# Illumina/strelka

Measured on AMD Instinct MI355X. Metric: candidate-alignment scoring cells/s (read bases x candidate alignments; Strelka2 has no pair-HMM, SURVEY.md section 0) + germline loci/s + 40x WGS-like germline wall-clock (e2e) + 110x/40x somatic wall-clock (e2e_somatic), higher is better.
Workload: dtype f64; 1 GPU; germline chr20-style synthetic (BASELINE.json configs[1]).  Headline: scoreCandidateAlignment as one function -- per GPU per step 65536 reads of 150 bp x 87.9 candidate alignments each (5-7 candidate indels around them), from the candidate alignments the device search left (PCal) to one double each: one kernel (F5: the walk of each alignment's path + the terms of its bases, penalties and clips).  ; read_len=150

## Files before the change

### include/strelka_amd.h

```cpp
#ifndef STRELKA_AMD_H
#define STRELKA_AMD_H

#include <stddef.h>
#include <stdint.h>

#ifdef __cplusplus
extern "C" {
#endif

#define SK_VERSION 100


int sk_device_count(void);
void* sk_host_alloc(size_t bytes);
void sk_host_free(void* p);
int sk_init(int device);
int sk_init_strict(int device);
void sk_shutdown(void);
const char* sk_last_error(void);
int sk_version(void);
int sk_is_initialized(void);
int sk_sync_mode(void);
int sk_libm_restated(void);

int sk_broker_client(void);
int sk_broker_enable(int on);
int sk_broker_serve(int device, const char* socket_name, int idle_seconds);
int sk_broker_selftest(int n, uint32_t mul);

int sk_check_device_errors(void);

int sk_debug_set_g3_variant(int variant);
int sk_debug_g3_global_pass_count(void);
int sk_debug_force_device_libm(int on);
void sk_debug_region_alleles(int no_edge_deletion, int ids_twice);

int sk_get_qscore_tables(double* q2p, double* q2lncompe, double* q2lne);


enum { SK_BAM_REF = 0, SK_BAM_A = 1, SK_BAM_C = 2, SK_BAM_G = 4, SK_BAM_T = 8, SK_BAM_ANY = 15 };

enum {
    SK_OP_BASES = 0,
    SK_OP_SOFT_CLIP = 1,
    SK_OP_NOBASE = 2
};
enum { SK_OPFLAG_NONCANDIDATE_PENALTY = 1 };

typedef struct sk_score_op {
    uint16_t length;
// ... 836 lines not shown
```

### strelka_amd/capi.py

```python
import ctypes as C
import os

import numpy as np

_HERE = os.path.dirname(os.path.abspath(__file__))
LIB_PATH = os.path.join(_HERE, "lib", "libstrelka_amd.so")

c_void_p = C.c_void_p


class ScoreOp(C.Structure):
    _fields_ = [("length", C.c_uint16), ("kind", C.c_uint8), ("flags", C.c_uint8), ("src", C.c_int32)]


SCORE_OP_DTYPE = np.dtype([("length", "<u2"), ("kind", "u1"), ("flags", "u1"), ("src", "<i4")])
OP_BASES, OP_SOFT_CLIP, OP_NOBASE = 0, 1, 2
OPFLAG_PENALTY = 1


class AlignBatch(C.Structure):
    _fields_ = [("n_reads", C.c_int32), ("n_cals", C.c_int32), ("n_ops", C.c_int64),
                ("read_off", c_void_p), ("read_code", c_void_p), ("read_qual", c_void_p),
                ("hap_off", c_void_p), ("hap_code", c_void_p), ("cal_off", c_void_p), ("op_off", c_void_p),
                ("ops", c_void_p), ("max_read_len", C.c_int32), ("max_hap_len", C.c_int32),
# ... 198 lines not shown
    "sk_score_alignments", "sk_score_alignments_dev", "sk_align_evmask_words", "sk_align_prepare", "sk_align_colmat_words", "sk_align_prepare_cols",
    "sk_bgzf_scan", "sk_bgzf_inflate", "sk_bgzf_inflate_prefixed", "sk_bgzf_inflate_dev", "sk_bgzf_deflate_bound", "sk_bgzf_deflate", "sk_bgzf_deflate_dev", "sk_bam_header_end", "sk_bam_scan_records", "sk_bam_decode", "sk_bam_decode_kept", "sk_bam_decode_dev", "sk_normalize_alignments", "sk_normalize_alignments_dev",
    "sk_intake_options_default", "sk_read_intake_obs_bound", "sk_read_intake", "sk_read_intake_dev", "sk_read_intake_scratch_bytes",
    "sk_ar_state_initial", "sk_ref_anchors", "sk_ref_anchors_dev", "sk_active_regions_bound", "sk_active_regions", "sk_active_regions_dev",
    "sk_region_haplotypes_seq_bound", "sk_region_haplotypes_support_bound", "sk_region_haplotypes_scratch_bytes", "sk_region_haplotypes", "sk_region_haplotypes_dev",
    "sk_region_alleles_allele_bound", "sk_region_alleles_insert_bound", "sk_region_alleles_scratch_bytes", "sk_region_alleles", "sk_region_alleles_dev", "sk_debug_region_alleles",
    "sk_align_builder_create", "sk_align_builder_destroy", "sk_align_builder_clear", "sk_align_builder_append", "sk_align_builder_add_read",
    "sk_align_builder_finish", "sk_align_builder_error", "sk_align_builder_set_host_threads",
    "sk_align_scores_default", "sk_global_align",
    "sk_pileup_options_default", "sk_pileup_reads", "sk_pileup_reads_dev", "sk_pileup_scratch_bytes",
    "sk_pileup_stream_create", "sk_pileup_stream_destroy", "sk_pileup_stream_begin_region", "sk_pileup_stream_push", "sk_pileup_stream_push_begin", "sk_pileup_stream_push_finish", "sk_pileup_stream_enable_evs_words", "sk_gvcf_site_summaries", "sk_gvcf_site_summaries_dev", "sk_gvcf_plain_runs_dev", "sk_gvcf_plain_runs", "sk_pileup_stream_set_gvcf_block_options",
    "sk_somatic_pileup_stream_create", "sk_somatic_pileup_stream_destroy", "sk_somatic_pileup_stream_begin_region", "sk_somatic_pileup_stream_push", "sk_somatic_pileup_stream_push_begin", "sk_somatic_pileup_stream_push_finish",
    "sk_realign_options_default", "sk_realign_job_create", "sk_realign_job_destroy", "sk_realign_job_error",
    "sk_realign_job_set_reference", "sk_realign_job_set_indels", "sk_realign_job_add_read", "sk_realign_job_add_reads", "sk_realign_job_get_batch",
    "sk_realign_job_finish", "sk_realign_job_run", "sk_realign_job_n_reads", "sk_realign_job_read_result",
    "sk_realign_job_clear_reads", "sk_realign_job_rescore", "sk_realign_job_indels_consulted", "sk_realign_job_enumeration_counts", "sk_realign_device_job_counts", "sk_realign_reference_reads_outside", "sk_realign_job_stage3_counts", "sk_make_start_pos_alignment", "sk_get_end_pin_start_pos",
    "sk_germline_options_default", "sk_dependent_eprob", "sk_dependent_eprob_dev", "sk_site_digt_call",
    "sk_site_digt_call_dev", "sk_site_digt_call_fused", "sk_site_digt_call_fused_dev",
    "sk_somatic_snv_options_default", "sk_somatic_snv_call_batch", "sk_somatic_snv_call_batch_dev",
    "sk_somatic_snv_call_tiers", "sk_somatic_snv_call_tiers_dev", "sk_somatic_snv_tiers_scratch_bytes",
    "sk_indel_options_default", "sk_somatic_indel_options_default", "sk_indel_grid_lhood", "sk_indel_grid_lhood_dev",
    "sk_somatic_indel_call_batch", "sk_somatic_indel_call_tiers", "sk_allele_group_genotype_lhoods", "sk_allele_group_genotype_lhoods_dev",
    "sk_allele_group_genotype_lhoods_wide", "sk_allele_group_genotype_lhoods_wide_dev",
    "sk_allele_group_genotype_lhoods_xwide", "sk_allele_group_genotype_lhoods_xwide_dev",
    "sk_discover_indels_and_mismatches", "sk_global_align_scratch_bytes", "sk_global_align_dev", "sk_bai_query", "sk_bam_region_filter", "sk_gvcf_block_sites", "sk_gvcf_block_sites_dev",
]

_lib = None


def lib():
# ... 19 lines not shown
        L.sk_align_scores_default.argtypes = [C.POINTER(AlignScores)]
        L.sk_global_align.argtypes = [C.POINTER(GlobalAlignBatch), C.POINTER(AlignScores), c_void_p, c_void_p, c_void_p, c_void_p]
        L.sk_pileup_options_default.argtypes = [C.POINTER(PileupOptions)]
        L.sk_pileup_reads.argtypes = [C.POINTER(ReadBatchStruct), C.POINTER(PileupOptions), C.c_int, C.POINTER(PileupColumns)]
        L.sk_pileup_scratch_bytes.restype = C.c_int64
        L.sk_pileup_scratch_bytes.argtypes = [C.c_int32, C.c_int64, C.c_int32]
        L.sk_pileup_reads_dev.argtypes = [C.POINTER(ReadBatchStruct), C.c_int64, C.POINTER(PileupOptions), C.c_int,
                                          C.POINTER(PileupColumns), c_void_p, c_void_p]
        L.sk_realign_options_default.argtypes = [C.POINTER(RealignOptions)]
        L.sk_realign_job_create.restype = c_void_p
        L.sk_realign_job_create.argtypes = [C.POINTER(RealignOptions)]
        L.sk_realign_job_destroy.argtypes = [c_void_p]
        L.sk_realign_job_enumeration_counts.argtypes = [c_void_p, c_void_p, c_void_p, c_void_p]
        L.sk_realign_device_job_counts.argtypes = [c_void_p, c_void_p, c_void_p]
        L.sk_realign_device_job_counts.restype = None
        L.sk_realign_reference_reads_outside.argtypes = []
        L.sk_realign_reference_reads_outside.restype = C.c_int64
        L.sk_realign_job_stage3_counts.argtypes = [c_void_p, c_void_p, c_void_p]
        L.sk_realign_job_indels_consulted.argtypes = [c_void_p, c_void_p, C.c_int32]
        L.sk_realign_job_error.restype = C.c_char_p
        L.sk_realign_job_error.argtypes = [c_void_p]
        L.sk_realign_job_set_reference.argtypes = [c_void_p, C.c_char_p, C.c_int32, C.c_int32]
        L.sk_realign_job_set_indels.argtypes = [c_void_p, C.POINTER(IndelInfo), C.c_int32]
        L.sk_realign_job_add_read.argtypes = [c_void_p, C.POINTER(ReadInput)]
        L.sk_realign_job_add_reads.argtypes = [c_void_p, C.POINTER(ReadInput), C.c_int32]
        L.sk_realign_job_get_batch.argtypes = [c_void_p, C.POINTER(AlignBatch)]
        L.sk_realign_job_finish.argtypes = [c_void_p, c_void_p]
        L.sk_realign_job_run.argtypes = [c_void_p]
        L.sk_realign_job_n_reads.argtypes = [c_void_p]
        L.sk_realign_job_read_result.argtypes = [c_void_p, C.c_int32, C.POINTER(ReadResult)]
# ... 682 lines not shown
        if lib().sk_realign_job_indels_consulted(self._j, _p(out), self._n_indels):
            raise self._err()
        return out[:self._n_indels]

    def enumeration_counts(self):
        a, b, c = C.c_int64(), C.c_int64(), C.c_int64()
        lib().sk_realign_job_enumeration_counts(self._j, C.byref(a), C.byref(b), C.byref(c))
        return a.value, b.value, c.value

    @staticmethod
    def device_job_counts():
        a, b, c = C.c_int64(), C.c_int64(), C.c_int64()
        lib().sk_realign_device_job_counts(C.byref(a), C.byref(b), C.byref(c))
        return a.value, b.value, c.value

    def stage3_counts(self):
        a, b = C.c_int64(), C.c_int64()
        lib().sk_realign_job_stage3_counts(self._j, C.byref(a), C.byref(b))
        return a.value, b.value

    def clear_reads(self):
        lib().sk_realign_job_clear_reads(self._j)

    def result(self, i):
        r = ReadResult()
        if lib().sk_realign_job_read_result(self._j, i, C.byref(r)):
            raise StrelkaAmdError("bad read index")
        scores = []
        for q in range(r.n_scores):
            s = r.scores[q]
# ... 696 lines not shown
```

### strelka_amd/csrc/read_enumerate.hip

```cpp

#include "sk_common.h"

#include "align_entry.h"
#include "read_enumerate.h"

#include <algorithm>
#include <chrono>
#include <climits>
#include <cstdio>
#include <cstdlib>
#include <cstring>
#include <vector>

using namespace skcore;

int sk_score_alignments_launch_hostleg(const sk_align_batch* b, double* dev_out_lnp, void* hip_stream);

namespace
{

static_assert(sizeof(PFrame) % 4 == 0 && sizeof(PCal) % 4 == 0, "frames move through LDS as 32-bit words");


struct EnumArgs
// ... 238 lines not shown


enum { DYN_N_GROUPED = 0, DYN_N_CALS, DYN_N_LIGHT, DYN_N_HEAVY, DYN_FLAGS, DYN_MAX_CALS, DYN_REF_OUTSIDE, DYN_COUNT = 8 };
enum { DYNF_DEEPER = 1,
       DYNF_POOL_FULL = 2 };
enum { SEARCH_LEVELS = Caps::K + 2,
       CNT_LEVELS = 0,
       CNT_LEAVES = Caps::K + 3,
       CNT_NODES = (Caps::K + 5) & ~1,
       CNT_UNHANDLED = Caps::K + 7,
       CNT_DYN = Caps::K + 8,
       CNT_QUEUE = CNT_DYN + DYN_COUNT,
       N_COUNTERS = CNT_QUEUE + 2 };
static_assert(CNT_LEVELS + SEARCH_LEVELS + 1 == CNT_LEAVES && CNT_NODES > CNT_LEAVES && CNT_NODES + 2 <= CNT_UNHANDLED, "the counters' slots overlap");

__device__ inline int block_exclusive_scan(const int v, int* wave_sums , int* total)
{
    const int lane = threadIdx.x & 63, wave = threadIdx.x >> 6, n_waves = blockDim.x >> 6;
    int x = v;
    for (int d = 1; d < 64; d <<= 1) {
        const int y = __shfl_up(x, d);
        if (lane >= d) x += y;
    }
    __syncthreads();
    if (lane == 63) wave_sums[wave] = x;
    __syncthreads();
    if (threadIdx.x == 0) {
        int run = 0;
        for (int w = 0; w < n_waves; ++w) {
            const int t = wave_sums[w];
            wave_sums[w] = run;
            run += t;
        }
        wave_sums[n_waves] = run;
    }
    __syncthreads();
    *total = wave_sums[n_waves];
    return wave_sums[wave] + x - v;
}

struct ScanArgs
{
    int32_t n_reads;
    const int32_t* status;
    const int32_t* count;
// ... 448 lines not shown
constexpr int F5_TAB = 32;

static_assert(F5_TAB <= 32, "the table copy is a lane an entry, the consulted mask a bit an entry");

struct FusedScoreArgs
{
    FlatArgs f;
    const uint8_t* read_qual;
    const SkTables* tab;
    double* scores;
    unsigned* err;
    int32_t* n_unhandled;
    int32_t write_cals;
    unsigned long long* dbg;
    unsigned* queue;
};

constexpr int F5_SEGS = 16, F5_INDELS = 8;
constexpr int F5_STAMPS = 9;
constexpr int F5_SLOT = (F5_SEGS + 1) | 1;
__device__ __forceinline__ int f5_ent_word(const int k) { return k; }
constexpr int F5_ROW = 3;

struct F5Tab
{
    int32_t pos;
    uint32_t del, ins_len;
    uint32_t type_cand;
    int32_t ins_at;
};

template <int MAXR>
struct F5Lds
{
// ... 604 lines not shown
        const unsigned long long td = now();
        stamp[4] += td - tc;
        if (has && !bad) {
            const double lnp = f5_sum(S, myslot, n_ent, ln_noncand, ln_quarter);
            fa.scores[c0 + my_j] = lnp;
        }
        if (cons_mine && cons_seen == 0) a.job.consulted[tab_lo + lane] = 1;
        raw0.q0 = raw0.q1 = raw0.q2 = raw0.q3 = raw0.q4 = make_uint4(0, 0, 0, 0);
        raw0.i0 = raw0.i1 = raw0.i2 = raw0.i3 = 0;
        stamp[5] += now() - td;
    }
    if (TIMING && fa.dbg && lane == 0) {
        stamp[6] = now();
        stamp[3] = TIMING ? (unsigned long long)wall_clock64() - wall0 : 0ull;
        stamp[8] = draw_cycles;
        for (int i = 0; i < F5_STAMPS; ++i) fa.dbg[size_t(r) * F5_STAMPS + i] = stamp[i];
    }
}

template <int MAXR, bool TIMING, int WAVES>
__global__ __launch_bounds__(64 * WAVES) __attribute__((amdgpu_waves_per_eu(4, 4))) void flatten_score_kernel(const FusedScoreArgs fa, const int n_reads)
{
    __shared__ __attribute__((aligned(16))) F5Lds<MAXR> S[WAVES];
    __shared__ double q_terms[F5_Q_TERMS];
    for (int i = threadIdx.x; i < F5_Q_TERMS; i += 64 * WAVES) q_terms[i] = (i <= SK_NQ) ? fa.tab->q2lncompe[i] : fa.tab->q2mis[i - (SK_NQ + 1)];
    __syncthreads();
    const int wave = threadIdx.x >> 6, lane = threadIdx.x & 63;
    const unsigned n_waves = gridDim.x * unsigned(WAVES);
    unsigned r = blockIdx.x * unsigned(WAVES) + unsigned(wave);
    unsigned long long draw_cycles = 0;
    while (r < unsigned(n_reads)) {
        f5_read<MAXR, TIMING>(fa, int(r), S[wave], q_terms, draw_cycles);
        f5_wave_sync();
        const unsigned long long t0 = TIMING ? (unsigned long long)clock64() : 0ull;
        unsigned d = 0;
        if (lane == 0) d = atomicAdd(&fa.queue[0], 1u);
        int drawn = __builtin_amdgcn_readfirstlane(int(d));
        if (TIMING) __asm__ volatile("" : "+s"(drawn));
        r = n_waves + unsigned(drawn);
        draw_cycles = TIMING ? (unsigned long long)clock64() - t0 : 0ull;
    }
    if (lane == 0) {
        __threadfence();
        if (atomicAdd(&fa.queue[1], 1u) == gridDim.x * unsigned(WAVES) - 1u) {
            fa.queue[0] = 0u;
            fa.queue[1] = 0u;
        }
    }
}

template <int MAXR, bool TIMING>
static void launch_flatten_score_t(const int n_reads, hipStream_t st, const FusedScoreArgs& fs)
{
    static const int waves = [] { const char* e = std::getenv("SK_F5_WAVES"); return e ? std::atoi(e) : 0; }();
    constexpr int DEFAULT_WAVES = (sizeof(F5Lds<MAXR>) * 16 <= 160 * 1024) ? 8 : 4;
    const int w = waves > 0 ? waves : DEFAULT_WAVES;
    static const int grid_env = [] { const char* e = std::getenv("SK_F5_GRID"); return e ? std::atoi(e) : 0; }();
    constexpr int WAVES_PER_CU = int((160 * 1024) / sizeof(F5Lds<MAXR>)) >= 16 ? 16 : int((160 * 1024) / sizeof(F5Lds<MAXR>));
    auto grid = [&](const int wpb) {
        const int resident = grid_env > 0 ? grid_env : 256 * std::max(1, WAVES_PER_CU / wpb);
        return dim3(unsigned(std::max(1, std::min(resident, (n_reads + wpb - 1) / wpb))));
    };
    if (w == 16 && MAXR <= 152) SK_LAUNCH((flatten_score_kernel<152, TIMING, 16>), grid(16), dim3(1024), 0, st, fs, n_reads);
    else if (w >= 8) SK_LAUNCH((flatten_score_kernel<MAXR, TIMING, 8>), grid(8), dim3(512), 0, st, fs, n_reads);
    else if (w == 4) SK_LAUNCH((flatten_score_kernel<MAXR, TIMING, 4>), grid(4), dim3(256), 0, st, fs, n_reads);
    else if (w == 2) SK_LAUNCH((flatten_score_kernel<MAXR, TIMING, 2>), grid(2), dim3(128), 0, st, fs, n_reads);
    else SK_LAUNCH((flatten_score_kernel<MAXR, TIMING, 1>), grid(1), dim3(64), 0, st, fs, n_reads);
}

static void launch_flatten_score(const int n_reads, hipStream_t st, const FusedScoreArgs& fs)
{
    const bool short_reads = fs.f.max_read_len <= 152, timing = fs.dbg != nullptr;
    if (short_reads && !timing) launch_flatten_score_t<152, false>(n_reads, st, fs);
    else if (short_reads) launch_flatten_score_t<152, true>(n_reads, st, fs);
    else if (!timing) launch_flatten_score_t<F5_MAX_READ, false>(n_reads, st, fs);
    else launch_flatten_score_t<F5_MAX_READ, true>(n_reads, st, fs);
}

__global__ __launch_bounds__(64) void gather_cals_kernel(const PCal* __restrict__ pool, const int32_t* __restrict__ list, const int32_t n_cals,
                                                         PCal* __restrict__ cals)
{
    constexpr int REC_DW = int(sizeof(PCal) / 4);
// ... 465 lines not shown

struct EnumBuffers
{
    DevBuf in_arena, zero_arena, minmax_arena, mask_arena;
    HostBuf h_in_arena, h_zero_arena;
    View tab, ins, toggle, ref, ref_code, ins_code, reads, read_off, read_code, read_qual, r2i, i2r, orig, map_level;
    View counters, status, warn, n_raw, hap_len, fill, n_uniq, consulted;
    View win_begin, ins_lo, win_end, ins_hi, evmask, addmask;
    View h_counters, h_status, h_warn, h_n_raw, h_hap_len, h_n_uniq, h_consulted;
    View cal_off_z, h_cal_off_z;
    DevBuf level_a, level_b, pool, leaf_read, leaf_hash;
    DevBuf raw_off, grouped, ghash, gkey, dup, sorted;
    DevBuf n_ops, win_len, n_ins, ins_idx, ins_off, n_seg8;
    DevBuf cal_off, hap_off, cals, hap_code, op_off, ops, entries, scores, colmat, colmat_off;
    DevBuf s3_order, s3_smooth, s3_flag, s3_rm_type, s3_rm_pos, s3_key, s3_sorted_score, s3_sorted_hash, s3_next_same, s3_range_end, s3_removed, s3_out, s3_list;
    HostBuf h_s3_out, h_s3_list;
    HostBuf h_raw_off, h_n_ops, h_cal_off, h_hap_off, h_op_off, h_cals, h_scores, h_colmat_off;
};
EnumBuffers& bufs()
{
    static EnumBuffers b;
    return b;
}

int reserve_dev(std::initializer_list<std::pair<DevBuf&, size_t>> wants)
{
    for (const auto& w : wants)
        if (w.first.reserve(std::max<size_t>(w.second, 256))) return 1;
    return 0;
}
// ... 60 lines not shown
    SK_HIP(skrt::setDevice(ctx.device));
    if (!g_cals_gathered) {
        if (bufs().cals.reserve(sizeof(PCal) * size_t(g_n_cals))) return 1;
        SK_LAUNCH(gather_cals_kernel, dim3((g_n_cals + 63) / 64), dim3(64), 0, ctx.stream, g_cals_pool, g_cals_list, g_n_cals, bufs().cals.as<PCal>());
        SK_HIP(skrt::getLastError());
        g_cals_gathered = true;
    }
    SK_HIP(skrt::memcpyAsync(dst, bufs().cals.as<PCal>() + first, sizeof(PCal) * size_t(count), hipMemcpyDeviceToHost, ctx.stream));
    SK_HIP(skrt::streamSynchronize(ctx.stream));
    return 0;
}

namespace
{
int64_t g_jobs_one_wait = 0, g_jobs_one_wait_redone = 0, g_jobs_staged = 0;
struct JobSeconds
{
    double setup = 0, submit = 0, wait = 0, after = 0;
    ~JobSeconds()
    {
        if (std::getenv("SK_ENUM_JOB_SECONDS"))
            std::fprintf(stderr, "strelka_amd enum job seconds: jobs=%lld setup=%.4f submit=%.4f wait=%.4f after=%.4f\n", (long long)g_jobs_one_wait, setup, submit,
                         wait, after);
    }
} g_job_seconds;
}
extern "C" void sk_enum_device_job_counts(int64_t* one_wait, int64_t* one_wait_redone, int64_t* staged)
{
    if (one_wait) *one_wait = g_jobs_one_wait;
    if (one_wait_redone) *one_wait_redone = g_jobs_one_wait_redone;
    if (staged) *staged = g_jobs_staged;
}

namespace
{
struct JobPlan
{
    const SkEnumInput* in = nullptr;
    EnumBuffers& B = bufs();
    hipStream_t st = nullptr;
    bool one_wait = false, with_stage3 = false;
    int n = 0;
    int64_t n_bases = 0, frame_cap = 0, pool_cap = 0;
    int W = 0;
    int max_order = 0;
    size_t in_bytes = 0, zero_bytes = 0, minmax_bytes = 0, mask_bytes = 0;
    size_t minmax_split = 0;
// ... 48 lines not shown
    if (one_wait && !(test_caps && test_caps[0])) p.pool_cap = std::min<int64_t>(p.pool_cap, std::max<int64_t>(int64_t(n) * 256, 1 << 17));
    const bool s3 = p.with_stage3 = in->want_scores && in->want_stage3;
    const int W = p.W = sk_ent_evmask_words(std::max(in->max_read_len, 0));
    for (int r = 0; r < n; ++r) p.max_order = std::max(p.max_order, int(in->reads[r].n_order));
    if (const char* e = std::getenv("SK_STAGE3_TEST_LDS_CALS")) {
        int a = 0, b = 0;
        if (std::sscanf(e, "%d,%d", &a, &b) == 2 && a > 0 && b >= a && b <= S3_LDS_CALS) {
            p.light_cals = a;
            p.lds_cals = b;
        }
    }
    if (reserve_dev({ { B.level_a, sizeof(PFrame) * size_t(p.frame_cap) }, { B.level_b, sizeof(PFrame) * size_t(p.frame_cap) },
                      { B.pool, sizeof(PCal) * size_t(p.pool_cap) }, { B.leaf_read, 4 * size_t(p.pool_cap) }, { B.leaf_hash, 4 * size_t(p.pool_cap) },
                      { B.raw_off, 4 * size_t(n + 1) }, { B.win_len, 4 * size_t(n) }, { B.n_ins, 4 * size_t(n) },
                      { B.ins_idx, 2 * size_t(n) * INS_CAP }, { B.ins_off, 4 * size_t(n) * INS_CAP },
                      { B.cal_off, 4 * size_t(n + 1) }, { B.hap_off, 8 * size_t(n + 1) } }) ||
        reserve_pinned({ { B.h_raw_off, 4 * size_t(n + 1) }, { B.h_cal_off, 4 * size_t(n + 1) }, { B.h_hap_off, 8 * size_t(n + 1) } }))
        return 1;
    Piece ins_p[] = {
        { &B.tab, in->tab, sizeof(PIndel) * size_t(in->n_tab), 0 },
        { &B.ins, in->ins_pool, size_t(in->ins_pool_len), 0 },
        { &B.toggle, in->max_toggle, sizeof(uint32_t) * size_t(in->n_max_toggle), 0 },
        { &B.ref, in->ref, size_t(std::max(in->ref_len, 0)), 0 },
        { &B.reads, in->reads, sizeof(PRead) * size_t(n), 0 },
        { &B.read_off, in->read_off, sizeof(int64_t) * size_t(n + 1), 0 },
        { &B.read_code, in->read_code, size_t(n_bases), 0 },
        { &B.read_qual, in->read_qual, size_t(n_bases), 0 },
        { &B.r2i, in->r2i, s3 ? 8 * size_t(in->n_tab) : 0, 0 },
        { &B.i2r, in->i2r, s3 ? 8 * size_t(in->n_tab) : 0, 0 },
        { &B.orig, in->orig, s3 ? 4 * size_t(in->n_tab) : 0, 0 },
        { &B.map_level, in->map_level, s3 ? 4 * size_t(n) : 0, 0 },
// ... 226 lines not shown
}

FusedScoreArgs fused_args(const JobPlan& p, const FlatArgs& fa)
{
    EnumBuffers& B = p.B;
    FusedScoreArgs fs;
    fs.f = fa;
    fs.read_qual = B.read_qual.as<uint8_t>();
    fs.tab = sk_ctx().dev_tables;
    fs.scores = B.scores.as<double>();
    fs.err = sk_ctx().dev_error_flags;
    fs.n_unhandled = B.counters.as<int32_t>() + CNT_UNHANDLED;
    fs.queue = B.counters.as<unsigned>() + CNT_QUEUE;
    fs.write_cals = 0;
    fs.dbg = nullptr;
    return fs;
}

int reserve_stage3(EnumBuffers& B, const int n, const int64_t n_bases, const int32_t n_cals)
{
    if (reserve_dev({ { B.s3_order, 4 * size_t(n_cals) }, { B.s3_smooth, 8 * size_t(n_cals) }, { B.s3_flag, size_t(n_cals) },
                      { B.s3_rm_type, size_t(n_bases) }, { B.s3_rm_pos, 4 * size_t(n_bases) }, { B.s3_key, 16 * size_t(n_cals) },
                      { B.s3_sorted_score, 8 * size_t(n_cals) }, { B.s3_sorted_hash, 4 * size_t(n_cals) }, { B.s3_next_same, 4 * size_t(n_cals) },
                      { B.s3_removed, size_t(n_cals) }, { B.s3_range_end, 4 * size_t(n_cals) }, { B.s3_out, sizeof(sk3::Out) * size_t(n) } }))
        return 1;
    return reserve_pinned({ { B.h_s3_out, sizeof(sk3::Out) * size_t(n) } });
}

Stage3Args stage3_args(const JobPlan& p, const FlatArgs& fa, const PCal* cals, const int32_t* slot, const int32_t* skip_if)
{
    EnumBuffers& B = p.B;
// ... 112 lines not shown
    sc.pool_cap = n_cap;
    SK_LAUNCH(job_scan_kernel<false>, dim3(1), dim3(1024), 0, st, sc);
    const SetArgs sa = set_args(p, n_cap, ea.n_leaves, B.cal_off_z.as<int32_t>());
    const int e2_blocks = int(std::min<int64_t>(std::max<int64_t>((int64_t(n) * 64 + 255) / 256, 8), 2048));
    SK_LAUNCH(group_kernel, dim3(e2_blocks), dim3(256), 0, st, sa);
    SK_LAUNCH(dedupe_kernel, dim3(e2_blocks), dim3(256), 0, st, sa);
    sc.count = B.n_uniq.as<int32_t>();
    sc.off = B.cal_off_z.as<int32_t>();
    sc.list = B.s3_list.as<int32_t>();
    sc.light_cals = p.light_cals;
    SK_LAUNCH(job_scan_kernel<true>, dim3(1), dim3(1024), 0, st, sc);
    SK_LAUNCH(rank_kernel, dim3(e2_blocks), dim3(256), 0, st, sa);
    const FlatArgs fa = flat_args(p, n_cap, true, B.cal_off_z.as<int32_t>(), nullptr, false);
    SK_LAUNCH(pool_bounds_kernel, dim3(e2_blocks), dim3(256), 0, st, fa);
    SK_LAUNCH(pool_layout_kernel, dim3((n + 63) / 64), dim3(64), 0, st, fa);
    const FusedScoreArgs fs = fused_args(p, fa);
    launch_flatten_score(n, st, fs);
    const Stage3Args s3 = stage3_args(p, fa, fa.pool, fa.list, fs.n_unhandled);
    launch_stage3<1>(st, s3, n, B.s3_list.as<int32_t>(), dyn + DYN_N_LIGHT, 1, p.light_cals);
    launch_stage3<4>(st, s3, n, B.s3_list.as<int32_t>() + (n - 1), dyn + DYN_N_HEAVY, -1, p.lds_cals);
    SK_HIP(skrt::getLastError());
    const size_t out_bytes = sizeof(sk3::Out) * size_t(n);
    if (stage_by_kernel()) {
        const uint32_t n_a = uint32_t(p.zero_bytes / 16), n_b = uint32_t((out_bytes + 15) / 16);
        const int blocks = int(std::min<size_t>(std::max<size_t>((std::max(p.zero_bytes, out_bytes) / 16 + 255) / 256, 1), 256));
        SK_LAUNCH(job_stage_out_kernel, dim3(blocks), dim3(256), 0, st, static_cast<const uint4*>(B.zero_arena.p), static_cast<uint4*>(B.h_zero_arena.p), n_a,
                  static_cast<const uint4*>(B.s3_out.p), static_cast<uint4*>(B.h_s3_out.p), n_b);
        SK_HIP(skrt::getLastError());
    } else {
        if (copy_down(st, B.h_zero_arena, B.zero_arena, p.zero_bytes) || copy_down(st, B.h_s3_out, B.s3_out, out_bytes)) return 1;
    }
// ... 231 lines not shown
    if (!p.with_stage3 && reserve_pinned({ { B.h_cals, sizeof(PCal) * size_t(n_cals) } })) return 1;
    const FlatArgs fa = flat_args(p, n_cals, false, B.cal_off.as<int32_t>(), B.n_ops.as<int32_t>(), false);
    SK_HIP(skrt::memsetAsync(B.minmax_arena.p, 0x7f, p.minmax_split, st));
    SK_HIP(skrt::memsetAsync(static_cast<char*>(B.minmax_arena.p) + p.minmax_split, 0x80, p.minmax_bytes - p.minmax_split, st));
    if (n_cals > 0) SK_LAUNCH(pool_bounds_kernel, dim3((n_cals + 255) / 256), dim3(256), 0, st, fa);
    SK_LAUNCH(pool_layout_kernel, dim3((n + 63) / 64), dim3(64), 0, st, fa);
    SK_HIP(skrt::getLastError());
    out->cals = B.h_cals.as<PCal>();
    g_n_cals = n_cals;
    g_cals_pool = fa.pool;
    g_cals_list = fa.list;

    const bool fused_enabled = !(std::getenv("SK_A5_FUSED") != nullptr && std::strcmp(std::getenv("SK_A5_FUSED"), "0") == 0);
    bool chain = !(fused_enabled && in->want_scores && n_cals > 0);
    if (!chain) {
        const FusedScoreArgs fs = fused_args(p, fa);
        launch_flatten_score(n, st, fs);
        SK_HIP(skrt::getLastError());
        p.lap("F5 flatten + score");
        if (in->want_stage3) {
            out->cals = nullptr;
        } else {
            if (reserve_dev({ { B.cals, sizeof(PCal) * size_t(n_cals) } })) return 1;
            SK_LAUNCH(gather_cals_kernel, dim3((n_cals + 63) / 64), dim3(64), 0, st, fa.pool, fa.list, n_cals, B.cals.as<PCal>());
            SK_HIP(skrt::getLastError());
            g_cals_gathered = true;
            if (copy_down(st, B.h_cals, B.cals, sizeof(PCal) * size_t(n_cals))) return 1;
        }
        remember_fused(p, fs, n_cals);
        if (after_scores(p, out, fa, false)) return 1;
        if (fetch_zero(p, B.counters, B.counters, 4 * size_t(N_COUNTERS))) return 1;
// ... 51 lines not shown
        first = std::min(first, s[0]);
        last = std::max(last, s[6]);
        sum[0] += double(s[1] - s[0]);
        for (int i = 2; i <= 5; ++i) sum[i] += double(s[i]);
        sum[7] += double(s[7]);
        sum[6] += double(s[6] - s[0]);
        sum[8] += double(s[8]);
        ndrawn += s[8] != 0;
    }
    for (const int grid : { 64, 256, 512, 1024, 1792, 2048, 4096 }) {
        if (grid > g_last.n) break;
        hipEvent_t a0, a1;
        SK_HIP(hipEventCreate(&a0));
        SK_HIP(hipEventCreate(&a1));
        FusedScoreArgs f2 = g_last.fs;
        launch_flatten_score(grid, st, f2);
        SK_HIP(hipEventRecord(a0, st));
        for (int k = 0; k < 5; ++k) launch_flatten_score(grid, st, f2);
        SK_HIP(hipEventRecord(a1, st));
        SK_HIP(hipEventSynchronize(a1));
        float ms = 0;
        SK_HIP(hipEventElapsedTime(&ms, a0, a1));
        std::fprintf(stderr, "[f5-timing] grid %d blocks: %.1f us per launch\n", grid, ms * 1000.f / 5.f);
        (void)hipEventDestroy(a0);
        (void)hipEventDestroy(a1);
    }
    if (nblk)
        std::fprintf(stderr, "[f5-timing] blocks %d: cycles per block: draw %.0f (%d drawn: %.0f each) prologue %.0f staging %.0f phaseA %.0f (walk %.0f) phaseB %.0f total %.0f = %.1f us by the 100 MHz counter (%.0f MHz); kernel span %llu cycles => %.1f blocks in flight\n",
                     nblk, sum[8] / nblk, ndrawn, sum[8] / std::max(1, ndrawn), sum[0] / nblk, sum[2] / nblk, sum[4] / nblk, sum[7] / nblk, sum[5] / nblk, sum[6] / nblk, sum[3] / nblk / 100.0,
                     sum[6] / std::max(1.0, sum[3]) * 100.0, last - first,
                     sum[6] / double(last - first));
    return 0;
}

extern "C" int sk_enum_device_rescore(const int32_t reps, float* out_ms, int32_t* out_n_reads, int32_t* out_n_cals, int64_t* out_cells)
{
    SK_REQUIRE_INIT();
    if (!g_last.valid) return sk_fail("sk_enum_device_rescore: no device run with scores to repeat");
    if (reps <= 0 || !out_ms) return sk_fail("sk_enum_device_rescore: bad argument");
    if (skrt::remote()) return sk_fail("sk_enum_device_rescore: a timing entry point (events); not carried by the broker -- unset STRELKA_AMD_BROKER");
    SkContext& ctx = sk_ctx();
    SK_HIP(skrt::setDevice(ctx.device));
    hipStream_t st = ctx.stream;
    EnumBuffers& B = bufs();
    const FlatArgs& fa = g_last.fa;
    hipEvent_t e0, e1;
// ... 30 lines not shown
```

Baseline: 847.9 billion cells/s.

## Reorder tail reads by candidate count to shorten F5 kernel drain

Adds a small kernel that builds a permutation for the last window of reads in the F5 flatten+score kernel. It bins reads by the number of 64-wide candidate chunks and shifts the heavy ones earlier in the hand-out order, so the final waves do not sit idle while a few long reads finish. The score kernel maps hand-out indices in that window through the table using readfirstlane. This costs one extra launch per job and an indirection per read, and the drain diagnostics gain a timing stamp.

```diff
diff --git a/include/strelka_amd.h b/include/strelka_amd.h
--- a/include/strelka_amd.h
+++ b/include/strelka_amd.h
@@ -34,6 +34,8 @@
 int sk_debug_g3_global_pass_count(void);
 int sk_debug_force_device_libm(int on);
 void sk_debug_region_alleles(int no_edge_deletion, int ids_twice);
+int sk_debug_f5_tail_order(const int32_t* cal_off, int32_t n_reads, int32_t waves, int32_t shift, int32_t* first, int32_t* n, int32_t* order_out);
+int64_t sk_debug_f5_tail_launches(void);
 
 int sk_get_qscore_tables(double* q2p, double* q2lncompe, double* q2lne);
 
diff --git a/strelka_amd/capi.py b/strelka_amd/capi.py
--- a/strelka_amd/capi.py
+++ b/strelka_amd/capi.py
@@ -236,7 +236,7 @@
     "sk_realign_options_default", "sk_realign_job_create", "sk_realign_job_destroy", "sk_realign_job_error",
     "sk_realign_job_set_reference", "sk_realign_job_set_indels", "sk_realign_job_add_read", "sk_realign_job_add_reads", "sk_realign_job_get_batch",
     "sk_realign_job_finish", "sk_realign_job_run", "sk_realign_job_n_reads", "sk_realign_job_read_result",
-    "sk_realign_job_clear_reads", "sk_realign_job_rescore", "sk_realign_job_indels_consulted", "sk_realign_job_enumeration_counts", "sk_realign_device_job_counts", "sk_realign_reference_reads_outside", "sk_realign_job_stage3_counts", "sk_make_start_pos_alignment", "sk_get_end_pin_start_pos",
+    "sk_realign_job_clear_reads", "sk_realign_job_rescore", "sk_realign_job_indels_consulted", "sk_realign_job_enumeration_counts", "sk_realign_device_job_counts", "sk_debug_f5_tail_order", "sk_debug_f5_tail_launches", "sk_realign_reference_reads_outside", "sk_realign_job_stage3_counts", "sk_make_start_pos_alignment", "sk_get_end_pin_start_pos",
     "sk_germline_options_default", "sk_dependent_eprob", "sk_dependent_eprob_dev", "sk_site_digt_call",
     "sk_site_digt_call_dev", "sk_site_digt_call_fused", "sk_site_digt_call_fused_dev",
     "sk_somatic_snv_options_default", "sk_somatic_snv_call_batch", "sk_somatic_snv_call_batch_dev",
@@ -286,6 +286,9 @@
         L.sk_realign_job_enumeration_counts.argtypes = [c_void_p, c_void_p, c_void_p, c_void_p]
         L.sk_realign_device_job_counts.argtypes = [c_void_p, c_void_p, c_void_p]
         L.sk_realign_device_job_counts.restype = None
+        L.sk_debug_f5_tail_order.argtypes = [c_void_p, C.c_int32, C.c_int32, C.c_int32, c_void_p, c_void_p, c_void_p]
+        L.sk_debug_f5_tail_launches.argtypes = []
+        L.sk_debug_f5_tail_launches.restype = C.c_int64
         L.sk_realign_reference_reads_outside.argtypes = []
         L.sk_realign_reference_reads_outside.restype = C.c_int64
         L.sk_realign_job_stage3_counts.argtypes = [c_void_p, c_void_p, c_void_p]
@@ -998,6 +1001,20 @@
         lib().sk_realign_device_job_counts(C.byref(a), C.byref(b), C.byref(c))
         return a.value, b.value, c.value
 
+    @staticmethod
+    def f5_tail_launches():
+        return int(lib().sk_debug_f5_tail_launches())
+
+    @staticmethod
+    def f5_tail_order(cal_off, waves, shift):
+        cal_off = np.ascontiguousarray(cal_off, np.int32)
+        n_reads = len(cal_off) - 1
+        first, n = C.c_int32(-1), C.c_int32(-1)
+        order = np.full(max(n_reads, 1), -2, np.int32)
+        if lib().sk_debug_f5_tail_order(_p(cal_off), n_reads, int(waves), int(shift), C.byref(first), C.byref(n), _p(order)):
+            raise StrelkaAmdError(last_error())
+        return first.value, order[:n.value].copy()
+
     def stage3_counts(self):
         a, b = C.c_int64(), C.c_int64()
         lib().sk_realign_job_stage3_counts(self._j, C.byref(a), C.byref(b))
diff --git a/strelka_amd/csrc/read_enumerate.hip b/strelka_amd/csrc/read_enumerate.hip
--- a/strelka_amd/csrc/read_enumerate.hip
+++ b/strelka_amd/csrc/read_enumerate.hip
@@ -276,21 +276,22 @@
        N_COUNTERS = CNT_QUEUE + 2 };
 static_assert(CNT_LEVELS + SEARCH_LEVELS + 1 == CNT_LEAVES && CNT_NODES > CNT_LEAVES && CNT_NODES + 2 <= CNT_UNHANDLED, "the counters' slots overlap");
 
-__device__ inline int block_exclusive_scan(const int v, int* wave_sums , int* total)
+template <typename V>
+__device__ inline V block_exclusive_scan(const V v, V* wave_sums , V* total)
 {
     const int lane = threadIdx.x & 63, wave = threadIdx.x >> 6, n_waves = blockDim.x >> 6;
-    int x = v;
+    V x = v;
     for (int d = 1; d < 64; d <<= 1) {
-        const int y = __shfl_up(x, d);
+        const V y = __shfl_up(x, d);
         if (lane >= d) x += y;
     }
     __syncthreads();
     if (lane == 63) wave_sums[wave] = x;
     __syncthreads();
     if (threadIdx.x == 0) {
-        int run = 0;
+        V run = 0;
         for (int w = 0; w < n_waves; ++w) {
-            const int t = wave_sums[w];
+            const V t = wave_sums[w];
             wave_sums[w] = run;
             run += t;
         }
@@ -769,10 +770,12 @@
     int32_t write_cals;
     unsigned long long* dbg;
     unsigned* queue;
+    const int32_t* tail_order;
+    uint32_t tail_first, tail_n;
 };
 
 constexpr int F5_SEGS = 16, F5_INDELS = 8;
-constexpr int F5_STAMPS = 9;
+constexpr int F5_STAMPS = 10;
 constexpr int F5_SLOT = (F5_SEGS + 1) | 1;
 __device__ __forceinline__ int f5_ent_word(const int k) { return k; }
 constexpr int F5_ROW = 3;
@@ -1407,6 +1410,7 @@
         stamp[6] = now();
         stamp[3] = TIMING ? (unsigned long long)wall_clock64() - wall0 : 0ull;
         stamp[8] = draw_cycles;
+        stamp[9] = wall0;
         for (int i = 0; i < F5_STAMPS; ++i) fa.dbg[size_t(r) * F5_STAMPS + i] = stamp[i];
     }
 }
@@ -1420,9 +1424,11 @@
     __syncthreads();
     const int wave = threadIdx.x >> 6, lane = threadIdx.x & 63;
     const unsigned n_waves = gridDim.x * unsigned(WAVES);
-    unsigned r = blockIdx.x * unsigned(WAVES) + unsigned(wave);
+    unsigned h = unsigned(__builtin_amdgcn_readfirstlane(int(blockIdx.x * unsigned(WAVES) + unsigned(wave))));
     unsigned long long draw_cycles = 0;
-    while (r < unsigned(n_reads)) {
+    while (h < unsigned(n_reads)) {
+        unsigned r = h;
+        if (h - fa.tail_first < fa.tail_n) r = unsigned(__builtin_amdgcn_readfirstlane(fa.tail_order[h - fa.tail_first]));
         f5_read<MAXR, TIMING>(fa, int(r), S[wave], q_terms, draw_cycles);
         f5_wave_sync();
         const unsigned long long t0 = TIMING ? (unsigned long long)clock64() : 0ull;
@@ -1430,7 +1436,7 @@
         if (lane == 0) d = atomicAdd(&fa.queue[0], 1u);
         int drawn = __builtin_amdgcn_readfirstlane(int(d));
         if (TIMING) __asm__ volatile("" : "+s"(drawn));
-        r = n_waves + unsigned(drawn);
+        h = n_waves + unsigned(drawn);
         draw_cycles = TIMING ? (unsigned long long)clock64() - t0 : 0ull;
     }
     if (lane == 0) {
@@ -1442,23 +1448,120 @@
     }
 }
 
-template <int MAXR, bool TIMING>
-static void launch_flatten_score_t(const int n_reads, hipStream_t st, const FusedScoreArgs& fs)
+struct F5Grid
+{
+    int wpb, blocks;
+    int waves() const { return wpb * blocks; }
+};
+template <int MAXR>
+static F5Grid f5_grid_t(const int n_reads)
 {
     static const int waves = [] { const char* e = std::getenv("SK_F5_WAVES"); return e ? std::atoi(e) : 0; }();
     constexpr int DEFAULT_WAVES = (sizeof(F5Lds<MAXR>) * 16 <= 160 * 1024) ? 8 : 4;
     const int w = waves > 0 ? waves : DEFAULT_WAVES;
+    const int wpb = (w == 16 && MAXR <= 152) ? 16 : w >= 8 ? 8 : w == 4 ? 4 : w == 2 ? 2 : 1;
     static const int grid_env = [] { const char* e = std::getenv("SK_F5_GRID"); return e ? std::atoi(e) : 0; }();
     constexpr int WAVES_PER_CU = int((160 * 1024) / sizeof(F5Lds<MAXR>)) >= 16 ? 16 : int((160 * 1024) / sizeof(F5Lds<MAXR>));
-    auto grid = [&](const int wpb) {
-        const int resident = grid_env > 0 ? grid_env : 256 * std::max(1, WAVES_PER_CU / wpb);
-        return dim3(unsigned(std::max(1, std::min(resident, (n_reads + wpb - 1) / wpb))));
-    };
-    if (w == 16 && MAXR <= 152) SK_LAUNCH((flatten_score_kernel<152, TIMING, 16>), grid(16), dim3(1024), 0, st, fs, n_reads);
-    else if (w >= 8) SK_LAUNCH((flatten_score_kernel<MAXR, TIMING, 8>), grid(8), dim3(512), 0, st, fs, n_reads);
-    else if (w == 4) SK_LAUNCH((flatten_score_kernel<MAXR, TIMING, 4>), grid(4), dim3(256), 0, st, fs, n_reads);
-    else if (w == 2) SK_LAUNCH((flatten_score_kernel<MAXR, TIMING, 2>), grid(2), dim3(128), 0, st, fs, n_reads);
-    else SK_LAUNCH((flatten_score_kernel<MAXR, TIMING, 1>), grid(1), dim3(64), 0, st, fs, n_reads);
+    const int resident = grid_env > 0 ? grid_env : 256 * std::max(1, WAVES_PER_CU / wpb);
+    return { wpb, std::max(1, std::min(resident, (n_reads + wpb - 1) / wpb)) };
+}
+static F5Grid f5_grid(const int n_reads, const int max_read_len)
+{
+    return max_read_len <= 152 ? f5_grid_t<152>(n_reads) : f5_grid_t<F5_MAX_READ>(n_reads);
+}
+
+template <int MAXR, bool TIMING>
+static void launch_flatten_score_t(const int n_reads, hipStream_t st, const FusedScoreArgs& fs)
+{
+    const F5Grid g = f5_grid_t<MAXR>(n_reads);
+    const dim3 grid(unsigned(g.blocks)), block(unsigned(64 * g.wpb));
+    if (g.wpb == 16) SK_LAUNCH((flatten_score_kernel<152, TIMING, 16>), grid, block, 0, st, fs, n_reads);
+    else if (g.wpb == 8) SK_LAUNCH((flatten_score_kernel<MAXR, TIMING, 8>), grid, block, 0, st, fs, n_reads);
+    else if (g.wpb == 4) SK_LAUNCH((flatten_score_kernel<MAXR, TIMING, 4>), grid, block, 0, st, fs, n_reads);
+    else if (g.wpb == 2) SK_LAUNCH((flatten_score_kernel<MAXR, TIMING, 2>), grid, block, 0, st, fs, n_reads);
+    else SK_LAUNCH((flatten_score_kernel<MAXR, TIMING, 1>), grid, block, 0, st, fs, n_reads);
+}
+
+constexpr int F5_TAIL_KINDS = 5;
+constexpr int F5_TAIL_MAX = 65536;
+struct TailArgs
+{
+    const int32_t* cal_off;
+    int32_t first, n;
+    int32_t shift;
+    int32_t* order;
+};
+__global__ __launch_bounds__(1024) void tail_order_kernel(const TailArgs a)
+{
+    constexpr int MAX_CHUNKS = F5_TAIL_MAX / 64, AHEAD = 8;
+    __shared__ unsigned long long mask[MAX_CHUNKS + 1][F5_TAIL_KINDS - 1];
+    __shared__ uint4 before[MAX_CHUNKS + 1];
+    __shared__ unsigned long long wave_sums[17];
+    const int T = a.n, t = threadIdx.x, lane = t & 63, wave = t >> 6;
+    const int n_chunks = (T + 63) >> 6;
+    for (int c0 = wave; c0 < n_chunks; c0 += 16 * AHEAD) {
+        int lo[AHEAD], hi[AHEAD];
+#pragma unroll
+        for (int u = 0; u < AHEAD; ++u) {
+            const int i = (c0 + 16 * u) * 64 + lane;
+            lo[u] = i < T ? a.cal_off[a.first + i] : 0;
+            hi[u] = i < T ? a.cal_off[a.first + i + 1] : 0;
+        }
+#pragma unroll
+        for (int u = 0; u < AHEAD; ++u) {
+            const int chunk = c0 + 16 * u;
+            if (chunk >= n_chunks) break;
+            const int kind = (chunk * 64 + lane < T) ? min(max((hi[u] - lo[u] + 63) >> 6, 1), F5_TAIL_KINDS) : 0;
+#pragma unroll
+            for (int q = 2; q <= F5_TAIL_KINDS; ++q) {
+                const unsigned long long m = __ballot(kind == q);
+                if (lane == 0) mask[chunk][q - 2] = m;
+            }
+        }
+    }
+    if (t < F5_TAIL_KINDS - 1) mask[n_chunks][t] = 0;
+    __syncthreads();
+    unsigned cnt[F5_TAIL_KINDS - 1] = { 0, 0, 0, 0 };
+    if (t < n_chunks) {
+#pragma unroll
+        for (int q = 0; q < F5_TAIL_KINDS - 1; ++q) cnt[q] = unsigned(__popcll(mask[t][q]));
+    }
+    unsigned long long tot23 = 0, tot45 = 0;
+    const unsigned long long at23 = block_exclusive_scan<unsigned long long>(cnt[0] | (unsigned long long)cnt[1] << 32, wave_sums, &tot23);
+    const unsigned long long at45 = block_exclusive_scan<unsigned long long>(cnt[2] | (unsigned long long)cnt[3] << 32, wave_sums, &tot45);
+    if (t < n_chunks) before[t] = make_uint4(unsigned(at23), unsigned(at23 >> 32), unsigned(at45), unsigned(at45 >> 32));
+    if (t == 0) before[n_chunks] = make_uint4(unsigned(tot23), unsigned(tot23 >> 32), unsigned(tot45), unsigned(tot45 >> 32));
+    __syncthreads();
+    for (int i = blockIdx.x * 1024 + t; i < T; i += gridDim.x * 1024) {
+        int c = 1;
+#pragma unroll
+        for (int q = 2; q <= F5_TAIL_KINDS; ++q)
+            if ((mask[i >> 6][q - 2] >> (i & 63)) & 1ull) c = q;
+        int place = 0;
+#pragma unroll
+        for (int q = 1; q <= F5_TAIL_KINDS; ++q) {
+            const long long x = (long long)i + (long long)(q - c) * a.shift + (q < c ? 1 : 0);
+            const int below = int(min(max(x, 0ll), (long long)T));
+            const uint4 p = before[below >> 6];
+            const unsigned long long bits = (1ull << (below & 63)) - 1ull;
+            const unsigned long long* const m = mask[below >> 6];
+            const unsigned n2 = p.x + unsigned(__popcll(m[0] & bits)), n3 = p.y + unsigned(__popcll(m[1] & bits));
+            const unsigned n4 = p.z + unsigned(__popcll(m[2] & bits)), n5 = p.w + unsigned(__popcll(m[3] & bits));
+            place += int(q == 1 ? unsigned(below) - (n2 + n3 + n4 + n5) : q == 2 ? n2 : q == 3 ? n3 : q == 4 ? n4 : n5);
+        }
+        if (unsigned(place) < unsigned(T)) a.order[place] = a.first + i;
+    }
+}
+static void launch_tail_order(hipStream_t st, const TailArgs& ta) { SK_LAUNCH(tail_order_kernel, dim3(unsigned(ta.n + 1023) / 1024), dim3(1024), 0, st, ta); }
+static int f5_tail_shift(const int W)
+{
+    static const int env = [] { const char* e = std::getenv("SK_F5_TAIL_SHIFT"); return e ? std::max(0, std::atoi(e)) : -1; }();
+    return std::min(env >= 0 ? env : W, std::max(0, (F5_TAIL_MAX - W) / 6));
+}
+static int f5_tail_window(const int n_reads, const int W, const int shift)
+{
+    if (n_reads <= W || shift <= 0) return 0;
+    return int(std::min<int64_t>(n_reads, int64_t(W) + 6 * int64_t(shift)));
 }
 
 static void launch_flatten_score(const int n_reads, hipStream_t st, const FusedScoreArgs& fs)
@@ -1954,6 +2057,7 @@
     DevBuf n_ops, win_len, n_ins, ins_idx, ins_off, n_seg8;
     DevBuf cal_off, hap_off, cals, hap_code, op_off, ops, entries, scores, colmat, colmat_off;
     DevBuf s3_order, s3_smooth, s3_flag, s3_rm_type, s3_rm_pos, s3_key, s3_sorted_score, s3_sorted_hash, s3_next_same, s3_range_end, s3_removed, s3_out, s3_list;
+    DevBuf tail_order;
     HostBuf h_s3_out, h_s3_list;
     HostBuf h_raw_off, h_n_ops, h_cal_off, h_hap_off, h_op_off, h_cals, h_scores, h_colmat_off;
 };
@@ -2044,6 +2148,7 @@
 namespace
 {
 int64_t g_jobs_one_wait = 0, g_jobs_one_wait_redone = 0, g_jobs_staged = 0;
+int64_t g_tail_launches = 0;
 struct JobSeconds
 {
     double setup = 0, submit = 0, wait = 0, after = 0;
@@ -2061,6 +2166,40 @@
     if (one_wait_redone) *one_wait_redone = g_jobs_one_wait_redone;
     if (staged) *staged = g_jobs_staged;
 }
+
+extern "C" int sk_debug_f5_tail_order(const int32_t* cal_off, const int32_t n_reads, const int32_t waves, const int32_t shift, int32_t* first, int32_t* n,
+                                      int32_t* order_out)
+{
+    SK_REQUIRE_INIT();
+    if (!cal_off || n_reads < 0 || waves <= 0 || !first || !n) return sk_fail("sk_debug_f5_tail_order: bad argument");
+    const int T = f5_tail_window(n_reads, waves, shift);
+    *first = T ? n_reads - T : 0;
+    *n = T;
+    if (T == 0) return 0;
+    if (T > F5_TAIL_MAX) return sk_fail("sk_debug_f5_tail_order: a window of more than 65536 hand-outs (the drivers cut the shift down)");
+    if (!order_out) return sk_fail("sk_debug_f5_tail_order: no room for the table");
+    SkContext& ctx = sk_ctx();
+    SK_HIP(skrt::setDevice(ctx.device));
+    hipStream_t st = ctx.stream;
+    int32_t *d_off = nullptr, *d_order = nullptr;
+    int rc = 0;
+    auto run = [&]() -> int {
+        SK_HIP(skrt::malloc_(&d_off, 4 * (size_t(n_reads) + 1)));
+        SK_HIP(skrt::malloc_(&d_order, 4 * size_t(T)));
+        SK_HIP(skrt::memcpyAsync(d_off, cal_off, 4 * (size_t(n_reads) + 1), hipMemcpyHostToDevice, st));
+        SK_HIP(skrt::memsetAsync(d_order, 0xff, 4 * size_t(T), st));
+        launch_tail_order(st, TailArgs{ d_off, n_reads - T, T, shift, d_order });
+        SK_HIP(skrt::getLastError());
+        SK_HIP(skrt::memcpyAsync(order_out, d_order, 4 * size_t(T), hipMemcpyDeviceToHost, st));
+        SK_HIP(skrt::streamSynchronize(st));
+        return 0;
+    };
+    rc = run();
+    if (d_off) (void)skrt::free_(d_off);
+    if (d_order) (void)skrt::free_(d_order);
+    return rc;
+}
+extern "C" int64_t sk_debug_f5_tail_launches(void) { return g_tail_launches; }
 
 namespace
 {
@@ -2139,7 +2278,8 @@
                       { B.pool, sizeof(PCal) * size_t(p.pool_cap) }, { B.leaf_read, 4 * size_t(p.pool_cap) }, { B.leaf_hash, 4 * size_t(p.pool_cap) },
                       { B.raw_off, 4 * size_t(n + 1) }, { B.win_len, 4 * size_t(n) }, { B.n_ins, 4 * size_t(n) },
                       { B.ins_idx, 2 * size_t(n) * INS_CAP }, { B.ins_off, 4 * size_t(n) * INS_CAP },
-                      { B.cal_off, 4 * size_t(n + 1) }, { B.hap_off, 8 * size_t(n + 1) } }) ||
+                      { B.cal_off, 4 * size_t(n + 1) }, { B.hap_off, 8 * size_t(n + 1) },
+                      { B.tail_order, 4 * size_t(std::min(n, F5_TAIL_MAX)) } }) ||
         reserve_pinned({ { B.h_raw_off, 4 * size_t(n + 1) }, { B.h_cal_off, 4 * size_t(n + 1) }, { B.h_hap_off, 8 * size_t(n + 1) } }))
         return 1;
     Piece ins_p[] = {
@@ -2396,7 +2536,22 @@
     fs.queue = B.counters.as<unsigned>() + CNT_QUEUE;
     fs.write_cals = 0;
     fs.dbg = nullptr;
+    fs.tail_order = nullptr;
+    fs.tail_first = fs.tail_n = 0;
     return fs;
+}
+
+void plan_tail(const JobPlan& p, FusedScoreArgs& fs)
+{
+    EnumBuffers& B = p.B;
+    const int W = f5_grid(p.n, fs.f.max_read_len).waves();
+    const int shift = f5_tail_shift(W), T = f5_tail_window(p.n, W, shift);
+    if (T == 0) return;
+    launch_tail_order(p.st, TailArgs{ fs.f.cal_off, p.n - T, T, shift, B.tail_order.as<int32_t>() });
+    ++g_tail_launches;
+    fs.tail_order = B.tail_order.as<int32_t>();
+    fs.tail_first = uint32_t(p.n - T);
+    fs.tail_n = uint32_t(T);
 }
 
 int reserve_stage3(EnumBuffers& B, const int n, const int64_t n_bases, const int32_t n_cals)
@@ -2539,7 +2694,8 @@
     const FlatArgs fa = flat_args(p, n_cap, true, B.cal_off_z.as<int32_t>(), nullptr, false);
     SK_LAUNCH(pool_bounds_kernel, dim3(e2_blocks), dim3(256), 0, st, fa);
     SK_LAUNCH(pool_layout_kernel, dim3((n + 63) / 64), dim3(64), 0, st, fa);
-    const FusedScoreArgs fs = fused_args(p, fa);
+    FusedScoreArgs fs = fused_args(p, fa);
+    plan_tail(p, fs);
     launch_flatten_score(n, st, fs);
     const Stage3Args s3 = stage3_args(p, fa, fa.pool, fa.list, fs.n_unhandled);
     launch_stage3<1>(st, s3, n, B.s3_list.as<int32_t>(), dyn + DYN_N_LIGHT, 1, p.light_cals);
@@ -2801,7 +2957,8 @@
     const bool fused_enabled = !(std::getenv("SK_A5_FUSED") != nullptr && std::strcmp(std::getenv("SK_A5_FUSED"), "0") == 0);
     bool chain = !(fused_enabled && in->want_scores && n_cals > 0);
     if (!chain) {
-        const FusedScoreArgs fs = fused_args(p, fa);
+        FusedScoreArgs fs = fused_args(p, fa);
+        plan_tail(p, fs);
         launch_flatten_score(n, st, fs);
         SK_HIP(skrt::getLastError());
         p.lap("F5 flatten + score");
@@ -2883,6 +3040,7 @@
         SK_HIP(hipEventCreate(&a0));
         SK_HIP(hipEventCreate(&a1));
         FusedScoreArgs f2 = g_last.fs;
+        f2.tail_n = 0;
         launch_flatten_score(grid, st, f2);
         SK_HIP(hipEventRecord(a0, st));
         for (int k = 0; k < 5; ++k) launch_flatten_score(grid, st, f2);
@@ -2899,6 +3057,22 @@
                      nblk, sum[8] / nblk, ndrawn, sum[8] / std::max(1, ndrawn), sum[0] / nblk, sum[2] / nblk, sum[4] / nblk, sum[7] / nblk, sum[5] / nblk, sum[6] / nblk, sum[3] / nblk / 100.0,
                      sum[6] / std::max(1.0, sum[3]) * 100.0, last - first,
                      sum[6] / double(last - first));
+    std::vector<std::pair<unsigned long long, unsigned long long>> span;
+    for (int r = 0; r < g_last.n; ++r) {
+        const unsigned long long* s = &h[size_t(r) * F5_STAMPS];
+        if (s[6] != 0) span.emplace_back(s[9], s[9] + s[3]);
+    }
+    if (!span.empty()) {
+        std::sort(span.begin(), span.end());
+        const unsigned long long w0 = span.front().first;
+        unsigned long long w1 = 0;
+        for (const auto& x : span) w1 = std::max(w1, x.second);
+        const size_t W = size_t(f5_grid(g_last.n, fs.f.max_read_len).waves()), n_last = std::min(W, span.size());
+        double idle = 0;
+        for (size_t i = span.size() - n_last; i < span.size(); ++i) idle += double(w1 - span[i].second);
+        std::fprintf(stderr, "[f5-timing] drain: tail window %u hand-outs; last read handed out at %.1f us, last read ended at %.1f us; over the %zu reads that started last a slot stood empty for %.1f us on average\n",
+                     fs.tail_n, double(span.back().first - w0) / 100.0, double(w1 - w0) / 100.0, n_last, idle / double(n_last) / 100.0);
+    }
     return 0;
 }
 
```

New measurement: 904.9 billion cells/s, median of 6. +6.7%, better.
